# JOBR0/PerceiverIO_Pytorch

Hardware: AMD Instinct MI355X
Metric: samples/sec PerceiverIO fwd (ImageNet-224, 512x1024 latents, 8 blocks x 6 self-attends) (higher is better)
Workload: dtype f16; 1 GPU; imagenet224 ClassificationPerceiver (conv+Fourier prep -> encoder 3136x322->512x1024, 8x6 SA -> decoder 1000 queries -> final Linear), all rows computed; batch_per_gpu=32, global_batch=32, precision_policy=fp16x2w/fp16sd/fp16x2af, parallelism=dp1 (batch sharded, all-gather of logits), launch=one HIP graph replay per step

## Files before the change

perceiverio_pytorch_amd/csrc/pio_flash.hip:

```cpp
#include <stdio.h>
#include <stdlib.h>

#include <type_traits>

#include "pio_internal.h"

namespace pio {

#ifndef PIO_FLASH_DEFAULT_VARIANT
#define PIO_FLASH_DEFAULT_VARIANT 0
#endif

struct FlashParams {
    const void *Q, *K, *VT;
    void *O;
    int Tq, Tk, H, nqt;
    int64_t ldq, ldk, ldvt, ldo;
    int64_t sQb, sKb, sVb, sOb;
    float scale_log2;
    int o_rows16;
};

static __device__ __attribute__((aligned(16))) uint32_t g_zero_chunk_f[4] = {0, 0, 0, 0};

template <int DV>
__device__ __forceinline__ int vrow_swz(int r) {
    if constexpr (DV == 128) return ((r & 3) << 2) | ((r >> 2) & 3);
    else if constexpr (DV == 64) return ((r >> 1) & 1) << 2;
    else return 0;
}

template <int DT, int DK, int DV, bool VROW, int NW, int KS = 1>
__global__ __launch_bounds__(NW * 64, NW >= 8 ? 1 : 2) void flash_attn_kernel(const FlashParams p) {
    typedef typename Op<DT>::T T;
    typedef typename Op<DT>::V8 V8;
    typedef typename Op<DT>::V4 V4;
    typedef short tr4 __attribute__((__vector_size__(4 * sizeof(short))));
    static_assert(!VROW || DV == 128 || DV == 64 || DV == 32 || DV == 160, "row-major V: swizzles exist for these widths");
    constexpr int KT = 64;
    constexpr int K_TILE = KT * DK * 2;
    constexpr int V_TILE = DV * KT * 2;
    constexpr int KCPR = DK / 8;
    constexpr int KRPB = 16 / KCPR;
    constexpr int K_PIECES = K_TILE / 1024;
    constexpr int V_PIECES = V_TILE / 1024;
    constexpr int NDT = DV / 32;
    constexpr int NQS = DK / 16;
    constexpr int OROW = DV * 2 + 16;
    static_assert(KS == 1 || ((KS == 2 || KS == 4) && NW == 4 * KS), "key split: KS groups of four waves");
    constexpr int NWQ = NW / KS;
    constexpr int MRG = KS > 1 ? (KS - 1) * NWQ * 64 * (NDT * 16 + 2) * 4 : 0;
    constexpr int RING = 2 * KS * (K_TILE + V_TILE), OSTG = NW * 32 * OROW;
    constexpr int SM0 = RING > OSTG ? RING : OSTG;
    __shared__ __attribute__((aligned(16))) char smem[SM0 > MRG ? SM0 : MRG];

    const int tid = threadIdx.x;
    const int lane = tid & 63;
    const int wave = __builtin_amdgcn_readfirstlane(tid >> 6);
    const int r32 = lane & 31, hh = lane >> 5;
    int bid = blockIdx.x;
    const int nblk = gridDim.x;
    if ((nblk & 7) == 0) bid = (bid & 7) * (nblk >> 3) + (bid >> 3);
    const int qt = bid % p.nqt, bh = bid / p.nqt;
    const int b = bh / p.H, h = bh % p.H;
    const int qb = KS == 1 ? wave : wave % NWQ, kh = KS == 1 ? 0 : wave / NWQ;
    const int q0 = qt * (NWQ * 32) + qb * 32;

    const T *Qg = (const T *)p.Q + b * p.sQb + (int64_t)h * DK;
    const T *Kg = (const T *)p.K + b * p.sKb + (int64_t)h * DK;
    const T *Vg = (const T *)p.VT + b * p.sVb + (VROW ? (int64_t)h * DV : (int64_t)h * DV * p.ldvt);
    const T *zsrc = (const T *)g_zero_chunk_f;

    V8 qf[NQS];

    const int ntiles_all = (p.Tk + KT - 1) / KT;
    const int ntiles = ntiles_all / KS;
    const int tile0 = kh * ntiles;

    auto stage = [&](int kt, int buf) {
        char *kb = smem + (buf * KS + kh) * (K_TILE + V_TILE);
        char *vb = kb + K_TILE;
        const int k0 = (tile0 + kt) * KT;
        for (int pc = qb; pc < K_PIECES; pc += NWQ) {
            const int row = pc * (64 / KCPR) + lane / KCPR;
            const int slot = lane % KCPR;
            const int c = slot ^ ((row / KRPB) & (KCPR - 1));
            int key = k0 + row;
            key = key < p.Tk ? key : p.Tk - 1;
            const T *src = Kg + (int64_t)key * p.ldk + c * 8;
            __builtin_amdgcn_global_load_lds((const __attribute__((address_space(1))) void *)src,
                                             (__attribute__((address_space(3))) void *)(kb + pc * 1024), 16, 0, 0);
        }
        if constexpr (VROW) {
            constexpr int VCPR = DV / 8;
            for (int pc = qb; pc < V_PIECES; pc += NWQ) {
                const int idx = pc * 64 + lane;
                const int row = idx / VCPR;
                const int slot = idx - row * VCPR;
                const int c = slot ^ vrow_swz<DV>(row);
                int key = k0 + row;
                key = key < p.Tk ? key : p.Tk - 1;
                const T *src = Vg + (int64_t)key * p.ldvt + c * 8;
                __builtin_amdgcn_global_load_lds((const __attribute__((address_space(1))) void *)src,
                                                 (__attribute__((address_space(3))) void *)(vb + pc * 1024), 16, 0,
                                                 0);
            }
        } else
        for (int pc = qb; pc < V_PIECES; pc += NWQ) {
            const int row = pc * 8 + (lane >> 3);
            const int slot = lane & 7;
            const int c = slot ^ ((row >> 1) & 7);
            const int kcol = k0 + c * 8;
            const T *src = (kcol < p.ldvt) ? Vg + (int64_t)row * p.ldvt + kcol : zsrc;
            __builtin_amdgcn_global_load_lds((const __attribute__((address_space(1))) void *)src,
                                             (__attribute__((address_space(3))) void *)(vb + pc * 1024), 16, 0, 0);
        }
    };

    f32x16 oacc[NDT];
#pragma unroll
    for (int i = 0; i < NDT; ++i)
#pragma unroll
        for (int j = 0; j < 16; ++j) oacc[i][j] = 0.f;
    float m_run = -INFINITY;
    float l_run = 0.f;

    int k_off[2];
#pragma unroll
    for (int t = 0; t < 2; ++t) k_off[t] = (32 * t + r32) * (DK * 2);
    const int k_swz = (r32 / KRPB) & (KCPR - 1);
    const int v_swz = (r32 >> 1) & 7;

    stage(0, 0);
    {
        int q = q0 + r32;
        q = q < p.Tq ? q : p.Tq - 1;
        const T *qrow = Qg + (int64_t)q * p.ldq + 8 * hh;
#pragma unroll
        for (int s = 0; s < NQS; ++s) qf[s] = *(const V8 *)(qrow + 16 * s);
    }
    for (int kt = 0; kt < ntiles; ++kt) {
        asm volatile("s_waitcnt vmcnt(0)" ::: "memory");
        __syncthreads();
        if (kt + 1 < ntiles) stage(kt + 1, (kt + 1) & 1);
        const char *kb = smem + ((kt & 1) * KS + kh) * (K_TILE + V_TILE);
        const char *vb = kb + K_TILE;

        f32x16 sacc[2];
#pragma unroll
        for (int t = 0; t < 2; ++t) {
#pragma unroll
            for (int j = 0; j < 16; ++j) sacc[t][j] = 0.f;
#pragma unroll
            for (int s = 0; s < NQS; ++s) {
                const int chunk = (2 * s + hh) ^ k_swz;
                const V8 kf = *(const V8 *)(kb + k_off[t] + chunk * 16);
                sacc[t] = Op<DT>::mfma32(kf, qf[s], sacc[t]);
            }
        }
        const bool tail = KS == 1 && (kt == ntiles - 1) && (p.Tk % KT != 0);
        float mx = -INFINITY;
        if (tail) {
#pragma unroll
            for (int t = 0; t < 2; ++t)
#pragma unroll
                for (int i = 0; i < 16; ++i) {
                    const int key = (tile0 + kt) * KT + 32 * t + (i & 3) + 8 * (i >> 2) + 4 * hh;
                    if (key >= p.Tk) sacc[t][i] = -INFINITY;
                }
        }
#pragma unroll
        for (int t = 0; t < 2; ++t)
#pragma unroll
            for (int i = 0; i < 16; ++i) mx = fmaxf(mx, sacc[t][i]);
        mx = fmaxf(mx, __shfl_xor(mx, 32, 64)) * p.scale_log2;
        const float m_new = fmaxf(m_run, mx);
        const float alpha = __builtin_amdgcn_exp2f(m_run - m_new);
        m_run = m_new;
        float psum = 0.f;
#pragma unroll
        for (int t = 0; t < 2; ++t)
#pragma unroll
            for (int i = 0; i < 16; ++i) {
                const float e = __builtin_amdgcn_exp2f(fmaf(sacc[t][i], p.scale_log2, -m_new));
                sacc[t][i] = e;
                psum += e;
            }
        l_run = l_run * alpha + psum;
        if (__builtin_amdgcn_ballot_w64(alpha != 1.0f) != 0) {
#pragma unroll
            for (int d = 0; d < NDT; ++d)
#pragma unroll
                for (int j = 0; j < 16; ++j) oacc[d][j] *= alpha;
        }

        V8 pf[2][2];
#pragma unroll
        for (int t = 0; t < 2; ++t)
#pragma unroll
            for (int s = 0; s < 2; ++s)
#pragma unroll
                for (int j = 0; j < 8; ++j) pf[t][s][j] = Op<DT>::from_f32(sacc[t][8 * s + j]);

#pragma unroll
        for (int d = 0; d < NDT; ++d) {
            const char *vrow = vb + (32 * d + r32) * 128;
#pragma unroll
            for (int t = 0; t < 2; ++t)
#pragma unroll
                for (int s = 0; s < 2; ++s) {
                    V4 lo, hi;
                    if constexpr (VROW) {
                        const int q4 = (lane & 15) >> 2, p4 = lane & 3, g1 = (lane >> 4) & 1;
                        const int chunk = d * 4 + 2 * g1 + (p4 >> 1);
#pragma unroll
                        for (int jj = 0; jj < 2; ++jj) {
                            const int key = 32 * t + 16 * s + 8 * jj + 4 * hh + q4;
                            const int f = vrow_swz<DV>(key);
                            const char *a = vb + key * (DV * 2) + ((chunk ^ f) << 4) + 8 * (p4 & 1);
                            const tr4 r = __builtin_amdgcn_ds_read_tr16_b64_v4i16(
                                (__attribute__((address_space(3))) tr4 *)a);
                            if (jj == 0) lo = __builtin_bit_cast(V4, r);
                            else hi = __builtin_bit_cast(V4, r);
                        }
                    } else {
                        const int g = 8 * t + 4 * s + hh;
                        lo = *(const V4 *)(vrow + ((((g >> 1)) ^ v_swz) << 4) + (g & 1) * 8);
                        hi = *(const V4 *)(vrow + ((((g + 2) >> 1) ^ v_swz) << 4) + (g & 1) * 8);
                    }
                    V8 vf;
#pragma unroll
                    for (int j = 0; j < 4; ++j) {
                        vf[j] = lo[j];
                        vf[4 + j] = hi[j];
                    }
                    oacc[d] = Op<DT>::mfma32(vf, pf[t][s], oacc[d]);
                }
        }
    }

    if constexpr (KS > 1) {
        __syncthreads();
        constexpr int MW = NDT * 16 + 2;
        if (kh > 0) {
            float *mg = (float *)smem + (size_t)(((kh - 1) * NWQ + qb) * 64 + lane) * MW;
#pragma unroll
            for (int d = 0; d < NDT; ++d)
#pragma unroll
                for (int j = 0; j < 16; ++j) mg[d * 16 + j] = oacc[d][j];
            mg[NDT * 16] = m_run;
            mg[NDT * 16 + 1] = l_run;
        }
        __syncthreads();
        if (kh == 0) {
#pragma unroll
            for (int part = 1; part < KS; ++part) {
                const float *mg = (const float *)smem + (size_t)(((part - 1) * NWQ + qb) * 64 + lane) * MW;
                const float m1 = mg[NDT * 16], l1 = mg[NDT * 16 + 1];
                const float m = fmaxf(m_run, m1);
                const float a0 = __builtin_amdgcn_exp2f(m_run - m), a1 = __builtin_amdgcn_exp2f(m1 - m);
#pragma unroll
                for (int d = 0; d < NDT; ++d)
#pragma unroll
                    for (int j = 0; j < 16; ++j) oacc[d][j] = oacc[d][j] * a0 + mg[d * 16 + j] * a1;
                l_run = l_run * a0 + l1 * a1;
                m_run = m;
            }
        }
    }
    const float l_tot = l_run + __shfl_xor(l_run, 32, 64);
    const float inv = 1.0f / l_tot;
    if (p.o_rows16) {
        __syncthreads();
        if (kh != 0) return;
        char *const ost = smem + qb * (32 * OROW);
        char *const orow = ost + r32 * OROW;
#pragma unroll
        for (int d = 0; d < NDT; ++d)
#pragma unroll
            for (int g4 = 0; g4 < 4; ++g4) {
                V4 o;
#pragma unroll
                for (int j = 0; j < 4; ++j) o[j] = Op<DT>::from_f32(oacc[d][4 * g4 + j] * inv);
                *(V4 *)(orow + (32 * d + 8 * g4 + 4 * hh) * 2) = o;
            }
        constexpr int CPR = DV / 8;
        T *const og = (T *)p.O + b * p.sOb + (int64_t)h * DV;
#pragma unroll
        for (int idx0 = 0; idx0 < 32 * CPR; idx0 += 64) {
            const int idx = idx0 + lane;
            const int row = idx / CPR, ch = idx % CPR;
            if (idx < 32 * CPR && q0 + row < p.Tq)
                *(V8 *)(og + (int64_t)(q0 + row) * p.ldo + ch * 8) = *(const V8 *)(ost + row * OROW + ch * 16);
        }
        return;
    }
    const int q = q0 + r32;
    if (q < p.Tq && kh == 0) {
        T *orow = (T *)p.O + b * p.sOb + (int64_t)q * p.ldo + (int64_t)h * DV;
#pragma unroll
        for (int d = 0; d < NDT; ++d)
#pragma unroll
            for (int g4 = 0; g4 < 4; ++g4) {
                V4 o;
#pragma unroll
                for (int j = 0; j < 4; ++j) o[j] = Op<DT>::from_f32(oacc[d][4 * g4 + j] * inv);
                *(V4 *)(orow + 32 * d + 8 * g4 + 4 * hh) = o;
            }
    }
}

#ifdef PIO_EXPERIMENTS
#include "../../tools/experiments/pio_flash_variants.inc"
#endif

bool flash_supported(int dkp, int dvp) {
    return (dkp == 128 && dvp == 128) || (dkp == 64 && dvp == 64) || (dkp == 32 && dvp == 32) ||
           (dkp == 32 && dvp == 160);
}

#ifdef PIO_EXPERIMENTS
int flash_variant_override(int which) {
    static int cur = [] {
        const char *e = getenv("PIO_FLASH_VARIANT");
        const int v = e ? atoi(e) : PIO_FLASH_DEFAULT_VARIANT;
        return (v >= 0 && v <= 2) ? v : PIO_FLASH_DEFAULT_VARIANT;
    }();
    const int prev = cur;
    if (which >= 0 && which <= 2) cur = which;
    return prev;
}
extern "C" int pio_debug_flash_variant(int which) { return flash_variant_override(which); }
#endif

int flash_attention_launch(int dtype, int dkp, int dvp, int dk_logical, const void *Q, const void *K, const void *VT,
                           void *O, int B, int H, int Tq, int Tk, int64_t ldq, int64_t ldk, int64_t ldvt, int64_t ldo,
                           int64_t sQb, int64_t sKb, int64_t sVb, int64_t sOb, bool v_rowmajor, hipStream_t s) {
    if (!flash_supported(dkp, dvp)) return PIO_E_SHAPE;
    if (!Q || !K || !VT || !O) return PIO_E_ARG;
    if (B <= 0 || H <= 0 || Tq <= 0 || Tk <= 0 || (int64_t)B * H * ((Tq + 127) / 128) > 0x7fffffffLL) return PIO_E_SHAPE;
    if ((ldq % 8) || (ldk % 8) || (ldvt % 8) || (ldo % 4) || (sQb % 8) || (sKb % 8) || (sVb % 8) || (sOb % 4))
        return PIO_E_ALIGN;
    if (((uintptr_t)Q & 15) || ((uintptr_t)K & 15) || ((uintptr_t)VT & 15) || ((uintptr_t)O & 7)) return PIO_E_ALIGN;
    const bool wide = v_rowmajor && Tq >= 256 && (int64_t)B * H * ((Tq + 255) / 256) >= 256;
    const int nqt = wide ? (Tq + 255) / 256 : (Tq + 127) / 128;
    const int o_rows16 = (ldo % 8 == 0 && sOb % 8 == 0 && ((uintptr_t)O & 15) == 0) ? 1 : 0;
    FlashParams p{Q, K, VT, O, Tq, Tk, H, nqt, ldq, ldk, ldvt, ldo, sQb, sKb, sVb, sOb,
                  1.4426950408889634f / sqrtf((float)dk_logical), o_rows16};
    dim3 grid((unsigned)(nqt * B * H), 1, 1);
    dim3 block(wide ? 512 : 256, 1, 1);
    ProfScope prof(PROF_FLASH, 2.0 * B * H * (double)Tq * Tk * (dkp + dvp),
                   2.0 * B * H * ((double)Tq * (dkp + dvp) + (double)Tk * (dkp + dvp)), s);
#define PIO_FLASH(DTV, DKV, DVV) hipLaunchKernelGGL((flash_attn_kernel<DTV, DKV, DVV, false, 4>), grid, block, 0, s, p)
#define PIO_FLASH_DT(DKV, DVV)                                         \
    do {                                                               \
        if (dtype == PIO_DT_F16) PIO_FLASH(PIO_DT_F16, DKV, DVV);      \
        else PIO_FLASH(PIO_DT_BF16, DKV, DVV);                         \
    } while (0)
#ifdef PIO_EXPERIMENTS
    const int variant = flash_variant_override(-2);
#else
    const int variant = 0;
#endif
    static const bool debug = [] {
        const char *e = getenv("PIO_FLASH_DEBUG");
        return e && atoi(e) != 0;
    }();
    if (debug)
        fprintf(stderr, "[pio] fused attention B=%d H=%d Tq=%d Tk=%d dkp=%d dvp=%d v_rowmajor=%d wide=%d variant=%d\n", B, H,
                Tq, Tk, dkp, dvp, (int)v_rowmajor, (int)wide, variant);
#ifdef PIO_EXPERIMENTS
    const bool pipe = variant == 1, stagger = variant == 2;
    if (v_rowmajor && Tq >= 256 && Tk % 128 == 0 && pipe && o_rows16) {
        FlashParams pp = p;
        pp.nqt = (Tq + 255) / 256;
        dim3 pgrid((unsigned)(pp.nqt * B * H), 1, 1);
        if (dtype == PIO_DT_F16) hipLaunchKernelGGL((flash_attn_pipe_kernel<PIO_DT_F16>), pgrid, dim3(256), 0, s, pp);
        else hipLaunchKernelGGL((flash_attn_pipe_kernel<PIO_DT_BF16>), pgrid, dim3(256), 0, s, pp);
    } else if (v_rowmajor && wide && stagger) {
        if (dtype == PIO_DT_F16) hipLaunchKernelGGL((flash_attn_stag_kernel<PIO_DT_F16>), grid, block, 0, s, p);
        else hipLaunchKernelGGL((flash_attn_stag_kernel<PIO_DT_BF16>), grid, block, 0, s, p);
    } else
#endif
    static const bool ksplit_on = [] {
        const char *e = getenv("PIO_FLASH_KSPLIT");
        return !e || atoi(e) != 0;
    }();
    const bool ksplit = ksplit_on && v_rowmajor && !wide && Tk >= 256 && (Tk % 128) == 0 &&
                        (int64_t)B * H * nqt <= cu_budget();
    const bool ksplit4 = ksplit && dkp <= 64 && dvp <= 64 && Tk >= 1024 && (Tk % 256) == 0;
    if (ksplit4) {
        block = dim3(1024, 1, 1);
        if (dkp == 64) {
            if (dtype == PIO_DT_F16) hipLaunchKernelGGL((flash_attn_kernel<PIO_DT_F16, 64, 64, true, 16, 4>), grid, block, 0, s, p);
            else hipLaunchKernelGGL((flash_attn_kernel<PIO_DT_BF16, 64, 64, true, 16, 4>), grid, block, 0, s, p);
        } else {
            if (dtype == PIO_DT_F16) hipLaunchKernelGGL((flash_attn_kernel<PIO_DT_F16, 32, 32, true, 16, 4>), grid, block, 0, s, p);
            else hipLaunchKernelGGL((flash_attn_kernel<PIO_DT_BF16, 32, 32, true, 16, 4>), grid, block, 0, s, p);
        }
    } else if (ksplit) {
        block = dim3(512, 1, 1);
#define PIO_FLASH_KS(DKV, DVV)                                                                                        \
    do {                                                                                                              \
        if (dtype == PIO_DT_F16)                                                                                      \
            hipLaunchKernelGGL((flash_attn_kernel<PIO_DT_F16, DKV, DVV, true, 8, 2>), grid, block, 0, s, p);          \
        else hipLaunchKernelGGL((flash_attn_kernel<PIO_DT_BF16, DKV, DVV, true, 8, 2>), grid, block, 0, s, p);        \
    } while (0)
        if (dkp == 128 && dvp == 128) PIO_FLASH_KS(128, 128);
        else if (dkp == 64 && dvp == 64) PIO_FLASH_KS(64, 64);
        else if (dkp == 32 && dvp == 32) PIO_FLASH_KS(32, 32);
        else PIO_FLASH_KS(32, 160);
#undef PIO_FLASH_KS
    } else if (v_rowmajor) {
#define PIO_FLASH_ROW(DKV, DVV)                                                                                        \
    do {                                                                                                               \
        if (wide) {                                                                                                    \
            if (dtype == PIO_DT_F16)                                                                                   \
                hipLaunchKernelGGL((flash_attn_kernel<PIO_DT_F16, DKV, DVV, true, 8>), grid, block, 0, s, p);          \
            else hipLaunchKernelGGL((flash_attn_kernel<PIO_DT_BF16, DKV, DVV, true, 8>), grid, block, 0, s, p);        \
        } else {                                                                                                       \
            if (dtype == PIO_DT_F16)                                                                                   \
                hipLaunchKernelGGL((flash_attn_kernel<PIO_DT_F16, DKV, DVV, true, 4>), grid, block, 0, s, p);          \
            else hipLaunchKernelGGL((flash_attn_kernel<PIO_DT_BF16, DKV, DVV, true, 4>), grid, block, 0, s, p);        \
        }                                                                                                              \
    } while (0)
        if (dkp == 128 && dvp == 128) PIO_FLASH_ROW(128, 128);
        else if (dkp == 64 && dvp == 64) PIO_FLASH_ROW(64, 64);
        else if (dkp == 32 && dvp == 32) PIO_FLASH_ROW(32, 32);
        else PIO_FLASH_ROW(32, 160);
#undef PIO_FLASH_ROW
    } else if (dkp == 128 && dvp == 128) PIO_FLASH_DT(128, 128);
    else if (dkp == 64 && dvp == 64) PIO_FLASH_DT(64, 64);
    else if (dkp == 32 && dvp == 32) PIO_FLASH_DT(32, 32);
    else PIO_FLASH_DT(32, 160);
#undef PIO_FLASH_DT
#undef PIO_FLASH
    return launch_status();
}

}
```

Measured before the change: 2003 samples/s.

## Add persistent flash-attention kernel with cross-block K/V prefetch and deferred output store

Adds a persistent flash-attention kernel for head dim 128. It launches one 512-thread workgroup per CU, and each workgroup loops over 256-query blocks. K/V tiles are double-buffered into LDS through global_load_lds, and the next block's first tile and Q fragments are prefetched while the current block finishes. The output store is deferred through LDS so it overlaps the next block's QK MFMAs. The goal is to remove tail effects and launch/prologue gaps between work tiles, at the cost of a single occupancy slot per CU and a new code path that is on by default.

```diff
diff --git a/perceiverio_pytorch_amd/csrc/pio_flash.hip b/perceiverio_pytorch_amd/csrc/pio_flash.hip
--- a/perceiverio_pytorch_amd/csrc/pio_flash.hip
+++ b/perceiverio_pytorch_amd/csrc/pio_flash.hip
@@ -310,6 +310,217 @@
     }
 }
 
+template <int DT>
+__global__ __launch_bounds__(512, 1) void flash_attn_persist_kernel(const FlashParams p, const int nblk) {
+    typedef typename Op<DT>::T T;
+    typedef typename Op<DT>::V8 V8;
+    typedef typename Op<DT>::V4 V4;
+    typedef short tr4 __attribute__((__vector_size__(4 * sizeof(short))));
+    constexpr int D = 128;
+    constexpr int KT = 64;
+    constexpr int TILE = KT * D * 2;
+    constexpr int OROW = D * 2 + 16;
+    __shared__ __attribute__((aligned(16))) char smem[4 * TILE + 8 * 32 * OROW];
+
+    const int tid = threadIdx.x;
+    const int lane = tid & 63;
+    const int wave = __builtin_amdgcn_readfirstlane(tid >> 6);
+    const int r32 = lane & 31, hh = lane >> 5;
+    char *const ost = smem + 4 * TILE + wave * (32 * OROW);
+
+    const int G = gridDim.x;
+    const int j0 = (G & 7) == 0 ? (int)(blockIdx.x & 7) * (G >> 3) + (int)(blockIdx.x >> 3) : (int)blockIdx.x;
+    const int ntiles = p.Tk / KT;
+    const int total = (nblk - j0 + G - 1) / G * ntiles;
+
+    struct Blk { int b, h, q0; };
+    auto blk = [&](int j) {
+        const int bh = j / p.nqt;
+        return Blk{bh / p.H, bh % p.H, (j % p.nqt) * 256 + wave * 32};
+    };
+
+    auto stage = [&](int j, int kt, int buf) {
+        const Blk k = blk(j);
+        const T *Kg = (const T *)p.K + k.b * p.sKb + (int64_t)k.h * D + (int64_t)kt * KT * p.ldk;
+        const T *Vg = (const T *)p.VT + k.b * p.sVb + (int64_t)k.h * D + (int64_t)kt * KT * p.ldvt;
+        char *kb = smem + buf * (2 * TILE);
+        char *vb = kb + TILE;
+#pragma unroll
+        for (int pc = wave; pc < TILE / 1024; pc += 8) {
+            const int row = pc * 4 + (lane >> 4);
+            const int c = (lane & 15) ^ (row & 15);
+            __builtin_amdgcn_global_load_lds((const __attribute__((address_space(1))) void *)(Kg + (int64_t)row * p.ldk + c * 8),
+                                             (__attribute__((address_space(3))) void *)(kb + pc * 1024), 16, 0, 0);
+        }
+#pragma unroll
+        for (int pc = wave; pc < TILE / 1024; pc += 8) {
+            const int row = pc * 4 + (lane >> 4);
+            const int c = (lane & 15) ^ vrow_swz<D>(row);
+            __builtin_amdgcn_global_load_lds((const __attribute__((address_space(1))) void *)(Vg + (int64_t)row * p.ldvt + c * 8),
+                                             (__attribute__((address_space(3))) void *)(vb + pc * 1024), 16, 0, 0);
+        }
+    };
+    auto load_q = [&](int j, V8 (&qd)[8]) {
+        const Blk k = blk(j);
+        int q = k.q0 + r32;
+        q = q < p.Tq ? q : p.Tq - 1;
+        const T *qrow = (const T *)p.Q + k.b * p.sQb + (int64_t)k.h * D + (int64_t)q * p.ldq + 8 * hh;
+#pragma unroll
+        for (int s = 0; s < 8; ++s) qd[s] = *(const V8 *)(qrow + 16 * s);
+    };
+    auto store_o = [&](int j) {
+        const Blk k = blk(j);
+        T *const og = (T *)p.O + k.b * p.sOb + (int64_t)k.h * D;
+#pragma unroll
+        for (int idx0 = 0; idx0 < 32 * 16; idx0 += 64) {
+            const int row = (idx0 + lane) >> 4, ch = lane & 15;
+            if (k.q0 + row < p.Tq)
+                *(V8 *)(og + (int64_t)(k.q0 + row) * p.ldo + ch * 8) = *(const V8 *)(ost + row * OROW + ch * 16);
+        }
+    };
+
+    V8 qf[8], qn[8];
+    f32x16 oacc[4];
+#pragma unroll
+    for (int i = 0; i < 4; ++i)
+#pragma unroll
+        for (int e = 0; e < 16; ++e) oacc[i][e] = 0.f;
+    float m_run = -INFINITY, l_run = 0.f;
+    const int k_swz = r32 & 15;
+    const int q4 = (lane & 15) >> 2, p4 = lane & 3, g1 = (lane >> 4) & 1;
+    uint32_t tr_off[2];
+#pragma unroll
+    for (int jj = 0; jj < 2; ++jj)
+        tr_off[jj] = (uint32_t)((8 * jj + 4 * hh + q4) * (D * 2) + (((2 * g1 + (p4 >> 1)) ^ (2 * jj + hh)) << 4) + 8 * (p4 & 1));
+
+    int j = j0, kt = 0;
+    int pend = -1;
+    stage(j0, 0, 0);
+    load_q(j0, qf);
+    for (int g = 0; g < total; ++g) {
+        asm volatile("s_waitcnt vmcnt(0)" ::: "memory");
+        __syncthreads();
+        const bool last = kt == ntiles - 1;
+        if (g + 1 < total) {
+            if (last) stage(j + G, 0, (g + 1) & 1);
+            else stage(j, kt + 1, (g + 1) & 1);
+        }
+        if (last && j + G < nblk) load_q(j + G, qn);
+        const char *kb = smem + (g & 1) * (2 * TILE);
+        const char *vb = kb + TILE;
+
+        f32x16 sacc[2];
+#pragma unroll
+        for (int t = 0; t < 2; ++t) {
+#pragma unroll
+            for (int e = 0; e < 16; ++e) sacc[t][e] = 0.f;
+#pragma unroll
+            for (int s = 0; s < 8; ++s) {
+                const int chunk = (2 * s + hh) ^ k_swz;
+                const V8 kf = *(const V8 *)(kb + (32 * t + r32) * (D * 2) + chunk * 16);
+                sacc[t] = Op<DT>::mfma32(kf, qf[s], sacc[t]);
+            }
+        }
+        if (pend >= 0) {
+            store_o(pend);
+            pend = -1;
+        }
+        float mx = -INFINITY;
+#pragma unroll
+        for (int t = 0; t < 2; ++t)
+#pragma unroll
+            for (int i = 0; i < 16; ++i) mx = fmaxf(mx, sacc[t][i]);
+        mx = fmaxf(mx, __shfl_xor(mx, 32, 64)) * p.scale_log2;
+        const float m_new = fmaxf(m_run, mx);
+        const float alpha = __builtin_amdgcn_exp2f(m_run - m_new);
+        m_run = m_new;
+        float psum = 0.f;
+#pragma unroll
+        for (int t = 0; t < 2; ++t)
+#pragma unroll
+            for (int i = 0; i < 16; ++i) {
+                const float e = __builtin_amdgcn_exp2f(fmaf(sacc[t][i], p.scale_log2, -m_new));
+                sacc[t][i] = e;
+                psum += e;
+            }
+        l_run = l_run * alpha + psum;
+        if (__builtin_amdgcn_ballot_w64(alpha != 1.0f) != 0) {
+#pragma unroll
+            for (int d = 0; d < 4; ++d)
+#pragma unroll
+                for (int e = 0; e < 16; ++e) oacc[d][e] *= alpha;
+        }
+        V8 pf[2][2];
+#pragma unroll
+        for (int t = 0; t < 2; ++t)
+#pragma unroll
+            for (int s = 0; s < 2; ++s)
+#pragma unroll
+                for (int e = 0; e < 8; ++e) pf[t][s][e] = Op<DT>::from_f32(sacc[t][8 * s + e]);
+
+#pragma unroll
+        for (int d = 0; d < 4; ++d) {
+#pragma unroll
+            for (int t = 0; t < 2; ++t)
+#pragma unroll
+                for (int s = 0; s < 2; ++s) {
+                    V4 h2[2];
+#pragma unroll
+                    for (int jj = 0; jj < 2; ++jj) {
+                        const char *a = vb + tr_off[jj] + ((d ^ q4) << 6) + (32 * t + 16 * s) * (D * 2);
+                        h2[jj] = __builtin_bit_cast(V4, __builtin_amdgcn_ds_read_tr16_b64_v4i16(
+                                                            (__attribute__((address_space(3))) tr4 *)a));
+                    }
+                    V8 vf;
+#pragma unroll
+                    for (int e = 0; e < 4; ++e) {
+                        vf[e] = h2[0][e];
+                        vf[4 + e] = h2[1][e];
+                    }
+                    oacc[d] = Op<DT>::mfma32(vf, pf[t][s], oacc[d]);
+                }
+        }
+
+        if (!last) {
+            ++kt;
+            continue;
+        }
+        const float inv = 1.0f / (l_run + __shfl_xor(l_run, 32, 64));
+        char *const orow = ost + r32 * OROW;
+#pragma unroll
+        for (int d = 0; d < 4; ++d)
+#pragma unroll
+            for (int g4 = 0; g4 < 4; ++g4) {
+                V4 o;
+#pragma unroll
+                for (int e = 0; e < 4; ++e) o[e] = Op<DT>::from_f32(oacc[d][4 * g4 + e] * inv);
+                *(V4 *)(orow + (32 * d + 8 * g4 + 4 * hh) * 2) = o;
+            }
+        pend = j;
+#pragma unroll
+        for (int d = 0; d < 4; ++d)
+#pragma unroll
+            for (int e = 0; e < 16; ++e) oacc[d][e] = 0.f;
+        m_run = -INFINITY;
+        l_run = 0.f;
+        if (j + G < nblk) {
+#pragma unroll
+            for (int s = 0; s < 8; ++s) qf[s] = qn[s];
+        }
+        j += G;
+        kt = 0;
+    }
+    if (pend >= 0) store_o(pend);
+}
+
+bool flash_persist_eligible(bool v_rowmajor, int dkp, int dvp, int Tq, int Tk, int o_rows16, int64_t nblk256, int cus) {
+    return v_rowmajor && dkp == 128 && dvp == 128 && Tq >= 256 && Tk % 64 == 0 && o_rows16 && nblk256 >= cus;
+}
+extern "C" int pio_debug_flash_persist_eligible(int v_rowmajor, int dkp, int dvp, int Tq, int Tk, int o_rows16,
+                                                int64_t nblk256, int cus) {
+    return flash_persist_eligible(v_rowmajor != 0, dkp, dvp, Tq, Tk, o_rows16, nblk256, cus) ? 1 : 0;
+}
+
 #ifdef PIO_EXPERIMENTS
 #include "../../tools/experiments/pio_flash_variants.inc"
 #endif
@@ -332,6 +543,17 @@
 }
 extern "C" int pio_debug_flash_variant(int which) { return flash_variant_override(which); }
 #endif
+
+static int flash_persist_override(int which) {
+    static int cur = [] {
+        const char *e = getenv("PIO_FLASH_PERSIST");
+        return (!e || atoi(e) != 0) ? 1 : 0;
+    }();
+    const int prev = cur;
+    if (which == 0 || which == 1) cur = which;
+    return prev;
+}
+extern "C" int pio_debug_flash_persist(int which) { return flash_persist_override(which); }
 
 int flash_attention_launch(int dtype, int dkp, int dvp, int dk_logical, const void *Q, const void *K, const void *VT,
                            void *O, int B, int H, int Tq, int Tk, int64_t ldq, int64_t ldk, int64_t ldvt, int64_t ldo,
@@ -366,9 +588,20 @@
         const char *e = getenv("PIO_FLASH_DEBUG");
         return e && atoi(e) != 0;
     }();
+    const int64_t nblk256 = (int64_t)B * H * ((Tq + 255) / 256);
+    const bool persist = flash_persist_override(-2) != 0 && variant == 0 &&
+                         flash_persist_eligible(v_rowmajor, dkp, dvp, Tq, Tk, o_rows16, nblk256, cu_budget());
     if (debug)
-        fprintf(stderr, "[pio] fused attention B=%d H=%d Tq=%d Tk=%d dkp=%d dvp=%d v_rowmajor=%d wide=%d variant=%d\n", B, H,
-                Tq, Tk, dkp, dvp, (int)v_rowmajor, (int)wide, variant);
+        fprintf(stderr, "[pio] fused attention B=%d H=%d Tq=%d Tk=%d dkp=%d dvp=%d v_rowmajor=%d wide=%d variant=%d persist=%d\n",
+                B, H, Tq, Tk, dkp, dvp, (int)v_rowmajor, (int)wide, variant, (int)persist);
+    if (persist) {
+        FlashParams pp = p;
+        pp.nqt = (Tq + 255) / 256;
+        const dim3 pgrid((unsigned)cu_budget(), 1, 1);
+        if (dtype == PIO_DT_F16) hipLaunchKernelGGL((flash_attn_persist_kernel<PIO_DT_F16>), pgrid, dim3(512), 0, s, pp, (int)nblk256);
+        else hipLaunchKernelGGL((flash_attn_persist_kernel<PIO_DT_BF16>), pgrid, dim3(512), 0, s, pp, (int)nblk256);
+        return launch_status();
+    }
 #ifdef PIO_EXPERIMENTS
     const bool pipe = variant == 1, stagger = variant == 2;
     if (v_rowmajor && Tq >= 256 && Tk % 128 == 0 && pipe && o_rows16) {
```

New measurement: 2025 samples/s, median of 6. 1.01x the previous value.
